# hermanjakobsen/robotic-ultrasound-imaging

Measured on AMD Instinct MI355X. Metric: env-steps/sec (whole node) at 4096 envs/GPU, random-action rollout, higher is better.
Workload: dtype f32

## Files before the change

robotic-ultrasound-imaging_amd/csrc/usim_step16.h:

```cpp
#pragma once
#include <type_traits>

namespace usim {

template <int N, class F>
DI void static_for(F&& f) {
    if constexpr (N > 0) { static_for<N - 1>(f); f(std::integral_constant<int, N - 1>{}); }
}

template <int CTRL>
DI float dpp0(float v) { return __int_as_float(__builtin_amdgcn_update_dpp(0, __float_as_int(v), CTRL, 0xf, 0xf, true)); }
template <int G> DI int glane() { return (int)(threadIdx.x & (G - 1)); }
template <int G, int K> DI float rbc(float v) {
    if constexpr (G == 16) return dpp0<0x150 + K>(v);
    else {
        const int iv = __float_as_int(v);
        const int t = __builtin_amdgcn_update_dpp(iv, iv, 0x150 + K, 0xf, 0x3, false);
        return __int_as_float(__builtin_amdgcn_update_dpp(t, iv, 0x150 + 8 + K, 0xf, 0xc, false));
    }
}
template <int G, int D> DI float rshr0(float v) {
    const float t = dpp0<0x110 + D>(v);
    if constexpr (G == 16) return t; else return (glane<G>() < D) ? 0.f : t;
}
// ... 93 lines not shown
            "v_fmac_f32_dpp %0, %3, %9 row_newbcast:%13 row_mask:0xf bank_mask:0xf\n\t" "v_fmac_f32_dpp %0, %4, %10 row_newbcast:%13 row_mask:0xf bank_mask:0xf\n\t"
            "v_fmac_f32_dpp %0, %5, %11 row_newbcast:%13 row_mask:0xf bank_mask:0xf\n\t" "v_fmac_f32_dpp %0, %6, %12 row_newbcast:%13 row_mask:0xf bank_mask:0xf"
            : "=&v"(s) : "v"(z.x), "v"(z.y), "v"(z.z), "v"(vo.x), "v"(vo.y), "v"(vo.z), "v"(n.x), "v"(n.y), "v"(n.z), "v"(f.x), "v"(f.y), "v"(f.z), "n"(K));
    } else {
        asm("s_nop 1\n\t"
            "v_mul_f32_dpp %0, %1, %7 row_newbcast:%13 row_mask:0xf bank_mask:0x3\n\t"   "v_mul_f32_dpp %0, %1, %7 row_newbcast:%14 row_mask:0xf bank_mask:0xc\n\t"
            "v_fmac_f32_dpp %0, %2, %8 row_newbcast:%13 row_mask:0xf bank_mask:0x3\n\t"  "v_fmac_f32_dpp %0, %2, %8 row_newbcast:%14 row_mask:0xf bank_mask:0xc\n\t"
            "v_fmac_f32_dpp %0, %3, %9 row_newbcast:%13 row_mask:0xf bank_mask:0x3\n\t"  "v_fmac_f32_dpp %0, %3, %9 row_newbcast:%14 row_mask:0xf bank_mask:0xc\n\t"
            "v_fmac_f32_dpp %0, %4, %10 row_newbcast:%13 row_mask:0xf bank_mask:0x3\n\t" "v_fmac_f32_dpp %0, %4, %10 row_newbcast:%14 row_mask:0xf bank_mask:0xc\n\t"
            "v_fmac_f32_dpp %0, %5, %11 row_newbcast:%13 row_mask:0xf bank_mask:0x3\n\t" "v_fmac_f32_dpp %0, %5, %11 row_newbcast:%14 row_mask:0xf bank_mask:0xc\n\t"
            "v_fmac_f32_dpp %0, %6, %12 row_newbcast:%13 row_mask:0xf bank_mask:0x3\n\t" "v_fmac_f32_dpp %0, %6, %12 row_newbcast:%14 row_mask:0xf bank_mask:0xc"
            : "=&v"(s) : "v"(z.x), "v"(z.y), "v"(z.z), "v"(vo.x), "v"(vo.y), "v"(vo.z), "v"(n.x), "v"(n.y), "v"(n.z), "v"(f.x), "v"(f.y), "v"(f.z), "n"(K), "n"(K + 8));
    }
    return s;
}

template <int G>
DI void fk16(const float* at, const float q, f3& X, f3& Y, f3& Z, f3& P) {
    float s, c;
    sincos_(q, s, c);
    const f3 f0 = mk(at[AT_RFIX], at[AT_RFIX + 1], at[AT_RFIX + 2]), f1 = mk(at[AT_RFIX + 3], at[AT_RFIX + 4], at[AT_RFIX + 5]);
    X = f0 * c + f1 * s; Y = f1 * c - f0 * s; Z = mk(at[AT_RFIX + 6], at[AT_RFIX + 7], at[AT_RFIX + 8]);
    P = mk(at[AT_LPOS], at[AT_LPOS + 1], at[AT_LPOS + 2]);
    static_for<3>([&](auto Dc) {
        constexpr int D = 1 << decltype(Dc)::value;
        const f3 LX = mk(rshr<G, D>(X.x, 1.f), rshr<G, D>(X.y, 0.f), rshr<G, D>(X.z, 0.f));
        const f3 LY = mk(rshr<G, D>(Y.x, 0.f), rshr<G, D>(Y.y, 1.f), rshr<G, D>(Y.z, 0.f));
        const f3 LZ = mk(rshr<G, D>(Z.x, 0.f), rshr<G, D>(Z.y, 0.f), rshr<G, D>(Z.z, 1.f));
        const f3 LP = mk(rshr0<G, D>(P.x), rshr0<G, D>(P.y), rshr0<G, D>(P.z));
        const f3 nX = LX * X.x + LY * X.y + LZ * X.z, nY = LX * Y.x + LY * Y.y + LZ * Y.z, nZ = LX * Z.x + LY * Z.y + LZ * Z.z;
        P = LP + LX * P.x + LY * P.y + LZ * P.z;
        X = nX; Y = nY; Z = nZ;
    });
}

DI void jacobian_rows(float* xl, const int gl, const float* Jc, float* Jr) {
    if (gl < 8) {
#pragma unroll
        for (int a = 0; a < 6; ++a) xl[a * 8 + gl] = Jc[a];
    }
    group_sync();
    int arow = (gl & 7) - ((gl & 4) ? 1 : 0);
    arow = arow > 5 ? 5 : arow;
    const float4 j0 = *reinterpret_cast<const float4*>(&xl[arow * 8]), j1 = *reinterpret_cast<const float4*>(&xl[arow * 8 + 4]);
    Jr[0] = j0.x; Jr[1] = j0.y; Jr[2] = j0.z; Jr[3] = j0.w; Jr[4] = j1.x; Jr[5] = j1.y; Jr[6] = j1.z; Jr[7] = j1.w;
}

template <int G>
DI float solve6_task(float* A, float b, const int gl) {
    static_for<6>([&](auto Kc) {
        constexpr int k = decltype(Kc)::value;
        constexpr int lk = TASK_LANE[k];
        const float g = (A[k] - (gl == lk ? 1.f : 0.f)) * rcp_(rbc<G, lk>(A[k]));
#pragma unroll
        for (int c = k + 1; c < 6; ++c) A[c] = fmaf(-g, rbc<G, lk>(A[c]), A[c]);
        b = fmaf(-g, rbc<G, lk>(b), b);
    });
    return b;
}

constexpr int X16_WORDS = 64;
constexpr int X16_RIGID_STRIDE = 84;

#ifndef USIM_WPR16
#define USIM_WPR16 4
#endif
#ifndef USIM_WPR8
#define USIM_WPR8 4
#endif
template <int G> constexpr int wpr() { return G == 16 ? USIM_WPR16 : USIM_WPR8; }
constexpr int MB_POSE = X16_WORDS;
constexpr int MB_OP = MB_POSE + 12;
constexpr int MB_W = MB_OP + 64;
constexpr int MB_Q = MB_W + 16;
constexpr int MB_GOAL = MB_Q + 100;
#ifndef USIM_DRAW_AHEAD
#define USIM_DRAW_AHEAD 1
#endif
constexpr bool DRAW_AHEAD = USIM_DRAW_AHEAD != 0;
#ifndef USIM_LIST_AHEAD
#define USIM_LIST_AHEAD 0
#endif
constexpr bool LIST_AHEAD = USIM_LIST_AHEAD != 0;
constexpr int MB_ACT = MB_GOAL + 12;
constexpr int X2_STRIDE = MB_ACT + (DRAW_AHEAD ? 8 : 0);
template <int G> constexpr int x2_base() { return TB_WORDS + (64 * wpr<G>() / G) * GE_STRIDE; }
static_assert(x2_base<16>() % 4 == 0 && x2_base<8>() % 4 == 0 && X2_STRIDE % 4 == 0 && MB_OP % 4 == 0 && MB_W % 4 == 0 && MB_ACT % 4 == 0, "mailbox block: 16-byte accesses");
static_assert((x2_base<8>() + 32 * X2_STRIDE) * 4 <= 160 * 1024, "split kernel with 8-lane groups: LDS of a CU");
#ifndef USIM_ARM_CULL16
#define USIM_ARM_CULL16 0
#endif
template <int G> constexpr int arm_cull_rounds() { return G == 16 ? USIM_ARM_CULL16 : 7; }

#if defined(USIM_TSTAMP) || defined(USIM_TSTAMP_NOWAIT)
#define USIM_BAR() do { __syncthreads(); ++nbar; } while (0)
#else
#define USIM_BAR() __syncthreads()
#endif


constexpr int ARM_LDS_WORDS = A16_LANES * AT_STRIDE;
template <int TORSO, int ROLE, int G> constexpr int arm_lds_base();
template <int NE, class WR = NoWarm>
struct Carry {
    float dqj, qdj, q0j;
    Episode ep;
    float s[NE], sd[NE];
    WR wr;
};

template <int TORSO, int ROLE, int G> constexpr int arm_lds_base() {
    return ROLE != 0 ? x2_base<G>() + (64 * wpr<G>() / G) * X2_STRIDE : (TORSO ? SOFT16_LDS_WORDS : 16 * X16_RIGID_STRIDE);
}
static_assert((arm_lds_base<1, 1, 8>() + ARM_LDS_WORDS) * 4 <= 160 * 1024 && arm_lds_base<1, 1, 8>() % 4 == 0 && arm_lds_base<1, 1, 16>() % 4 == 0 && arm_lds_base<1, 0, 16>() % 4 == 0
              && arm_lds_base<0, 0, 16>() % 4 == 0, "arm table behind the LDS blocks of every 16-lane kernel");

template <int TORSO, int MODE, int ROLE, int NT, int G = 16, bool RES = false, class WR = NoWarm, bool AHEAD = false>
DI void step16_one(float* lds, const DevModel& M, const DevCfg& C, float* __restrict__ st, const int n, const int npad, const DevIO& io, const int flags, const long long rstep,
                   const bool first_pass, const int sub, const bool more, int& nbar, Carry<TORSO ? (N_TOP + G - 1) / G : 1, WR>& cy) {
    static_assert(!AHEAD || (ROLE == 1 && RES), "action drawn ahead: the arm wave of a resident split launch");
    constexpr bool WARM = !std::is_same<WR, NoWarm>::value;
    static_assert(!WARM || (TORSO == 1 && ROLE == 0) || (TORSO == 1 && MODE == 0), "warm start: the soft-torso kernels");
    constexpr int WPR = (ROLE != 0) ? wpr<G>() : 4;
    constexpr int EPW = 64 / G, EPB = WPR * EPW;
    static_assert(!RES || MODE == 0, "resident state: step launches only");
    constexpr int X2_BASE = x2_base<G>();
    constexpr unsigned GMASK = (G == 16) ? 0xffffu : 0xffu;
    static_assert(G == 16 || (TORSO == 1 && MODE == 0 && ROLE != 0), "8-lane groups: the split soft-torso step only");
    constexpr int NE = TORSO ? (N_TOP + G - 1) / G : 1;
    static_assert(ROLE == 0 || (TORSO == 1 && MODE == 0), "the split kernel is the soft-torso step");
    const int lane = threadIdx.x & 63, wave = (threadIdx.x >> 6) & (WPR - 1);
    constexpr bool RES_HERE = RES && !(ROLE == 2 && G == 16);
    const bool fresh = !RES_HERE || first_pass;
    const int gl = lane & (G - 1), ge = lane / G;
    const int gbase = lane - gl;
    const int eb = wave * EPW + ge;
    const bool auto_reset = (flags & LF_AUTO_RESET) != 0;
    unsigned long long* const dbg = io.dbg;
    const bool refill = (MODE == 1) && io.refill != 0;
    const int item_cnt = refill ? io.count[0] : 1;
    const int item_first = refill ? (int)blockIdx.x * EPB : 0;
    for (int item0 = item_first; item0 < item_cnt; item0 += refill ? (int)gridDim.x * EPB : 1) {
    int env = blockIdx.x * EPB + eb;
    bool valid = env < n;
    int item_ep = 0;
    if (refill) {
        valid = item0 + eb < item_cnt;
        const int2 it = valid ? io.items[item0 + eb] : make_int2(0, 0);
        env = it.x; item_ep = it.y;
    }
    const bool store = valid && gl == 0;
    const int ei = valid ? env : (refill ? 0 : n - 1);
#define LAT(w) st[(size_t)F_LAT * npad + (size_t)ei * LAT_ENV_WORDS + (w)]
#define EB(off) lds[TB_WORDS + eb * GE_STRIDE + (off)]
    float* const warm_rows = st + warm_index(io.bank_row0, npad, (size_t)ei);
    int mbo = X2_BASE + eb * X2_STRIDE;
    if constexpr (ROLE != 0) asm volatile("" : "+v"(mbo));
    float* const xl = (ROLE != 0) ? &lds[mbo]
                                  : (TORSO ? &lds[TB_WORDS + eb * GE_STRIDE + GE_WS] : &lds[eb * X16_RIGID_STRIDE]);
    static_assert(GE_WS + X16_WORDS <= GE_STRIDE, "transpose scratch overlays the wrench records");
    constexpr int GOAL_OFF = (ROLE != 0) ? MB_GOAL : (TORSO ? GE_CG + (MAXCAND + 1) * CG_WORDS - GE_WS : X16_WORDS);
    static_assert(GE_CG + (MAXCAND + 1) * CG_WORDS + 12 <= GE_STRIDE && X16_WORDS + 12 <= X16_RIGID_STRIDE, "room for the goal");
    float* const goal_lds = xl + GOAL_OFF;

    USIM_STAMP(dbg, 0);
    if constexpr (ROLE == 1) { if (dbg && blockIdx.x == 0 && threadIdx.x == 0) dbg[20] = __builtin_readcyclecounter(); }

    float at[AT_STRIDE];
    {
        constexpr int ARM_LDS = arm_lds_base<TORSO, ROLE, G>();
        const float4* ap = fresh ? reinterpret_cast<const float4*>(M.tables + TB_ARM + gl * AT_STRIDE) : reinterpret_cast<const float4*>(lds + ARM_LDS + gl * AT_STRIDE);
        if (fresh) {
#pragma unroll
            for (int v = 0; v < AT_STRIDE / 4; ++v) { const float4 x = ap[v]; at[4 * v] = x.x; at[4 * v + 1] = x.y; at[4 * v + 2] = x.z; at[4 * v + 3] = x.w; }
            if constexpr (RES && ROLE != 2) {
                if (lane < G) {
#pragma unroll
                    for (int v = 0; v < AT_STRIDE / 4; ++v) reinterpret_cast<float4*>(lds + ARM_LDS + gl * AT_STRIDE)[v] = make_float4(at[4 * v], at[4 * v + 1], at[4 * v + 2], at[4 * v + 3]);
                }
            }
        } else {
            const float4* lp = reinterpret_cast<const float4*>(lds + ARM_LDS + gl * AT_STRIDE);
#pragma unroll
            for (int v = 0; v < AT_STRIDE / 4; ++v) { const float4 x = lp[v]; at[4 * v] = x.x; at[4 * v + 1] = x.y; at[4 * v + 2] = x.z; at[4 * v + 3] = x.w; }
        }
    }
    const float* const sp = st + scalar_index(0, (size_t)ei);
    const bool jlane = at[AT_JOINT] != 0.f;
    const int jl = jlane ? gl : NJ - 1;
    float &dqj = cy.dqj, &qdj = cy.qdj, &q0j = cy.q0j;
    Episode& E = cy.ep;
    f3 &ts = E.ts, &te = E.te;
    float &u0 = E.u0, &vbar = E.vbar, &fzbar = E.fzbar, &fzprev = E.fzprev, &dfz = E.dfz, &kst = E.kst, &kdmp = E.kdmp, &mu = E.mu, &epret = E.epret;
    int &t = E.t, &touched = E.touched, &episode = E.episode, &status = E.status;
    float (&s_pre)[NE] = cy.s, (&sd_pre)[NE] = cy.sd;
    if (fresh) {
        dqj = sp[F_Q + jl]; qdj = sp[F_QD + jl]; q0j = sp[F_Q0 + jl];
        float sv[20];
        {
            const float4* s4 = reinterpret_cast<const float4*>(sp + 20);
#pragma unroll
            for (int v = 0; v < 5; ++v) { const float4 x = s4[v]; sv[4 * v] = x.x; sv[4 * v + 1] = x.y; sv[4 * v + 2] = x.z; sv[4 * v + 3] = x.w; }
        }
#define SV(f) sv[(f) - 20]
        ts = mk(SV(F_TS), SV(F_TS + 1), SV(F_TS + 2)); te = mk(SV(F_TE), SV(F_TE + 1), SV(F_TE + 2));
        u0 = SV(F_U0); vbar = SV(F_VBAR); fzbar = SV(F_FZBAR); fzprev = SV(F_FZPREV); dfz = SV(F_DFZ);
        kst = SV(F_KST); kdmp = SV(F_KDMP); mu = SV(F_MU); epret = SV(F_EPRET);
        t = __float_as_int(SV(F_T)); touched = __float_as_int(SV(F_TOUCH)); episode = __float_as_int(SV(F_EPISODE)); status = __float_as_int(SV(F_STATUS));
#undef SV
#pragma unroll
        for (int i = 0; i < NE; ++i) {
            const int e = gl + i * G;
            s_pre[i] = 0.f; sd_pre[i] = 0.f;
            if (TORSO && MODE == 0 && ROLE != 1 && e < N_TOP) { s_pre[i] = LAT(LAT_S + e); sd_pre[i] = LAT(LAT_SD + e); }
            if (TORSO && MODE == 0 && ROLE == 1 && e < N_TOP) s_pre[i] = LAT(LAT_S + e);
        }
        if constexpr (WARM && MODE == 0 && ROLE != 1) warm_load(warm_rows, gl, cy.wr);
    } else if constexpr (RES && ROLE == 1) {
#pragma unroll
        for (int i = 0; i < NE; ++i) { const int e = gl + i * G; s_pre[i] = (e < N_TOP) ? EB(GE_S + e) : 0.f; }
    } else if constexpr (RES && ROLE == 2) {
        const float4 nx = *reinterpret_cast<const float4*>(&lds[mbo + MB_W]);
        if (nx.w != 0.f) {
            kst = nx.x; kdmp = nx.y; mu = nx.z; t = 0;
#pragma unroll
            for (int i = 0; i < NE; ++i) { s_pre[i] = 0.f; sd_pre[i] = 0.f; }
            warm_clear(cy.wr);
        }
    }
    if (!jlane) { dqj = 0.f; qdj = 0.f; q0j = 0.f; }
    float qj = q0j + dqj;
    if (TORSO != 0 && item0 == item_first && first_pass) {
        const float4* src = reinterpret_cast<const float4*>(M.tables);
        float4* dst = reinterpret_cast<float4*>(lds);
        constexpr int NV = TB_WORDS / 4, PER = (NV + NT - 1) / NT;
        float4 tmp[PER];
        int tix = threadIdx.x;
        asm volatile("" : "+v"(tix));
#pragma unroll
        for (int i = 0; i < PER; ++i) { int idx = tix + i * NT; tmp[i] = (idx < NV) ? src[idx] : make_float4(0, 0, 0, 0); }
#pragma unroll
        for (int i = 0; i < PER; ++i) { int idx = tix + i * NT; if (idx < NV) dst[idx] = tmp[i]; }
        USIM_BAR();
    }
    USIM_STAMP(dbg, 1);

    if (MODE == 0 && sub == 0) t += 1;
    const bool last_sub = sub == C.substeps - 1;
    const int tphys = (MODE == 0) ? (t - 1) * C.substeps + sub : 0;
    const float dt = C.dt, inv_h = rcp_((float)C.horizon);
#if defined(USIM_TSTAMP) || defined(USIM_TSTAMP_NOWAIT)
#define RSTAMP(k) do { if (dbg && blockIdx.x == 0 && (threadIdx.x & (64 * WPR - 1)) == 0) dbg[(ROLE == 2 ? 30 : 20) + (k)] = __builtin_readcyclecounter(); } while (0)
#else
#define RSTAMP(k) do { } while (0)
#endif
#define XSTAMP(k) RSTAMP(20 + (k))
    if constexpr (ROLE == 2) {
        RSTAMP(0);
        float* const mb = &lds[mbo];
        const int* tb_shell = reinterpret_cast<const int*>(lds + TB_SHELL);
        float dz, vz, az;
        torso_motion(C, tphys, dz, vz, az);
        lattice_rhs<G, NE>(lds, eb, gl, M, az, kst, kdmp, true, s_pre, sd_pre);
        lattice_solve<G>(lds, eb, gl, gbase);
        RSTAMP(1);
        USIM_BAR();
        RSTAMP(2);
        const f3 xs = mk(mb[MB_POSE], mb[MB_POSE + 1], mb[MB_POSE + 2]), sy = mk(mb[MB_POSE + 3], mb[MB_POSE + 4], mb[MB_POSE + 5]),
                 sz = mk(mb[MB_POSE + 6], mb[MB_POSE + 7], mb[MB_POSE + 8]);
        const f3 sxc = cross(sy, sz);
        int nq = __float_as_int(mb[MB_POSE + 10]);
#pragma unroll
        for (int i = arm_cull_rounds<G>(); i < NE; ++i) {
            const int eraw = i * G + gl, e = eraw < N_TOP ? eraw : N_TOP - 1;
            const bool cand = (eraw < N_TOP) && collide_cull(lds, e, M, C, s_pre[i], dz, xs, sxc, sz);
            const unsigned gm = (unsigned)(__ballot(cand) >> gbase) & GMASK;
            mb[MB_Q + (cand ? nq + __popc(gm & ((1u << gl) - 1u)) : 99)] = __int_as_float(e);
            nq += __popc(gm);
        }
        group_sync();
#if defined(USIM_TSTAMP) || defined(USIM_TSTAMP_NOWAIT)
        if (dbg && blockIdx.x == 0 && wave == 0 && gl == 0) dbg[54 + ge] = 1ull + (unsigned long long)nq;
#endif
        int nc = 0;
        collide_queue<G>(lds, mb + MB_Q, nq, &EB(GE_CG), gl, gbase, M, C, &EB(GE_S), dz, xs, sxc, sy, sz, nc);
        constexpr bool EARLY = G == 8;
        ContactRows P;
        constexpr bool LIST_EARLY = EARLY || (G == 16 && LIST_AHEAD);
        int nc_early = nc, overflow_early = 0, ncmax_early = 0, cel_early[MAXC];
        if constexpr (LIST_EARLY) {
            contact_overflow<G>(lds, eb, gl, gbase, nc_early);
            if (nc_early > MAXC) { overflow_early = 1; nc_early = MAXC; }
            group_sync();
            if constexpr (G == 16) {
                const int m01 = max(__builtin_amdgcn_readlane(nc_early, 0), __builtin_amdgcn_readlane(nc_early, 16));
                const int m23 = max(__builtin_amdgcn_readlane(nc_early, 32), __builtin_amdgcn_readlane(nc_early, 48));
                ncmax_early = max(m01, m23);
            } else {
#pragma unroll
                for (int k = MAXC; k >= 1; --k) if (ncmax_early == 0 && __any(nc_early >= k)) ncmax_early = k;
            }
#pragma unroll
            for (int k = 0; k < MAXC; ++k) cel_early[k] = (k < nc_early) ? __float_as_int(EB(GE_CG + k * CG_WORDS + 6)) : 0;
            if constexpr (EARLY) { if (ncmax_early > 0) contact_rows<G>(lds, eb, gl, M, C, nc_early, cel_early, vz, P); }
        }
        RSTAMP(3);
        USIM_BAR();
        RSTAMP(4);
        if constexpr (!LIST_EARLY) contact_overflow<G>(lds, eb, gl, gbase, nc);
        int overflow = 0;
        if (nc > MAXC) { overflow = 1; nc = MAXC; }
        if constexpr (!LIST_EARLY) group_sync();
        XSTAMP(0);
        int ncmax = 0;
        if constexpr (LIST_EARLY) { nc = nc_early; overflow = overflow_early; ncmax = ncmax_early; }
        else {
#pragma unroll
            for (int k = MAXC; k >= 1; --k) if (ncmax == 0 && __any(nc >= k)) ncmax = k;
        }
        XSTAMP(1);
        float gf[MAXC], W[6] = {0, 0, 0, 0, 0, 0};
        int cel[MAXC];
#pragma unroll
        for (int k = 0; k < MAXC; ++k) { const int ek = __float_as_int(EB(GE_CG + k * CG_WORDS + 6)); gf[k] = 0.f; cel[k] = LIST_EARLY ? cel_early[k] : ((k < nc) ? ek : 0); }
        if (ncmax > 0) {
            float alpha[6], vs[6], Lp[21];
#pragma unroll
            for (int a = 0; a < 6; ++a) {
                alpha[a] = mb[MB_OP + 48 + a]; vs[a] = mb[MB_OP + 54 + a];
#pragma unroll
                for (int b = 0; b <= a; ++b) Lp[PK(a, b)] = mb[MB_OP + a * 8 + b];
            }
            XSTAMP(2);
            contact_solve<G, EARLY, true>(lds, eb, gl, M, C, nc, ncmax, cel, Lp, alpha, vs, mu, vz, P, W, gf, dbg, cy.wr);
            XSTAMP(3);
        } else warm_clear(cy.wr);
        if (gl == 0) {
            *reinterpret_cast<float4*>(&mb[MB_W]) = make_float4(W[0], W[1], W[2], W[3]);
            *reinterpret_cast<float4*>(&mb[MB_W + 4]) = make_float4(W[4], W[5], __int_as_float(nc), __int_as_float(overflow));
#pragma unroll
            for (int k = 0; k < MAXC; ++k) { const int sh = tb_shell[cel[k]]; mb[MB_W + 8 + k] = __int_as_float((k < nc) ? sh : -1); }
        }
        RSTAMP(5);
        USIM_BAR();
        RSTAMP(6);
        {
            float acc_e[NE];
#pragma unroll
            for (int i = 0; i < NE; ++i) { const int e = gl + i * G; acc_e[i] = (e < N_TOP) ? EB(GE_A + e) : 0.f; }
#pragma unroll
            for (int k = 0; k < MAXC; ++k) {
#pragma unroll
                for (int i = 0; i < NE; ++i) {
                    const int e = (gl + i * G < N_TOP) ? gl + i * G : N_TOP - 1;
                    acc_e[i] = fmaf(lds[TB_LINV + e * LROW + cel[k]], gf[k], acc_e[i]);
                }
            }
#pragma unroll
            for (int i = 0; i < NE; ++i) {
                const int e = gl + i * G;
                if (e >= N_TOP) continue;
                const float sdn = sd_pre[i] + dt * acc_e[i];
                const float sn = s_pre[i] + dt * sdn;
                if (valid) { LAT(LAT_SD + e) = sdn; LAT(LAT_S + e) = sn; }
                if constexpr (RES) { sd_pre[i] = sdn; s_pre[i] = sn; EB(GE_S + e) = sn; }
            }
            if constexpr (WARM) { if (valid) warm_store(warm_rows, gl, cy.wr); }
        }
        RSTAMP(7);
        USIM_BAR();
        RSTAMP(8);
        return;
    }
    const int comp = gl & 3;
    const bool blk = (gl & 4) != 0;
    const bool is_task = (gl < 8) && comp != 3;
    auto pick = [&](f3 v) { return comp == 0 ? v.x : (comp == 1 ? v.y : v.z); };

    bool need = false;
    int ep_t = episode;
    if constexpr (MODE == 1) {
        need = refill ? valid : (io.mask ? io.mask[ei] != 0 : true);
        if (!__any(need)) continue;
        ep_t = refill ? item_ep : episode + 1;
        if (!refill) episode = ep_t;
        const uint32_t gid = (uint32_t)(C.env_offset + ei);
        const u4 r = philox(gid, (uint32_t)ep_t, (uint32_t)(gl < 3 ? gl : 2), 0u, C.key0, C.key1);
        const float ra = __uint_as_float(r.a), rb = __uint_as_float(r.b), rc = __uint_as_float(r.c), rd = __uint_as_float(r.d);
        u4 A, B, Cc;
        A.a = __float_as_uint(rbc<G, 0>(ra)); A.b = __float_as_uint(rbc<G, 0>(rb)); A.c = __float_as_uint(rbc<G, 0>(rc)); A.d = __float_as_uint(rbc<G, 0>(rd));
        B.a = __float_as_uint(rbc<G, 1>(ra)); B.b = __float_as_uint(rbc<G, 1>(rb)); B.c = __float_as_uint(rbc<G, 1>(rc)); B.d = __float_as_uint(rbc<G, 1>(rd));
        Cc.a = __float_as_uint(rbc<G, 2>(ra)); Cc.b = __float_as_uint(rbc<G, 2>(rb)); Cc.c = __float_as_uint(rbc<G, 2>(rc)); Cc.d = __float_as_uint(rbc<G, 2>(rd));
        const float tz = M.torso[2] + M.base[2] + C.top_off;
        f3 noise = mk(0, 0, 0);
        kst = C.stiffness; kdmp = C.damping;
        if (io.reset_params) {
            const float* p = io.reset_params + (size_t)ei * 13;
            ts = mk(p[0], p[1], p[2]); te = mk(p[3], p[4], p[5]); u0 = p[6]; noise = mk(p[7], p[8], p[9]);
            kst = p[10]; kdmp = p[11]; mu = p[12];
        } else {
            if (C.det_traj) { ts = mk(0.062f, -0.020f, 0.896f); te = mk(-0.032f, -0.075f, 0.896f); }
            else {
                const float tx = M.torso[0] + M.base[0], ty = M.torso[1] + M.base[1];
                const float xs0 = -0.15f + tx + 0.03f, xstep = (0.15f + tx - xs0) / 49.f;
                const float ys0 = -C.y_range + ty, ystep = 2.f * C.y_range / 49.f;
                ts = mk(xs0 + (float)urange(A.a, 50u) * xstep, ys0 + (float)urange(A.b, 50u) * ystep, tz);
                te = mk(xs0 + (float)urange(A.c, 50u) * xstep, ys0 + (float)urange(A.d, 50u) * ystep, tz);
            }
            u0 = u01(B.a);
            if (C.rand_pos) {
                const float r1 = sqrtf(-2.f * logf(u01_open(B.b))), th1 = 2.f * PI_F * u01(B.c);
                const float r2 = sqrtf(-2.f * logf(u01_open(B.d))), th2 = 2.f * PI_F * u01(Cc.a);
                noise = mk(r1 * cosf(th1) * 0.0025f, r1 * sinf(th1) * 0.0025f, r2 * cosf(th2) * 0.010f);
            }
            if (C.rand_solref) { kst = 1300.f + (float)urange(Cc.b, 300u); kdmp = 17.f + (float)urange(Cc.c, 24u); }
            float pf = C.probe_fric;
            if (C.rand_fric) pf *= 0.5f + 1.5f * u01(Cc.d);
            mu = fmaxf(pf, C.elem_fric);
            if (C.probe_geoms == 2 && !C.pair) mu = 0.5f * (mu + fmaxf(C.probe_fric2, C.elem_fric));
        }
        const float uu = clampf(u0, 0.f, 1.f);
        const f3 tp0 = ts + (te - ts) * uu;
        const f3 target = mk(tp0.x + noise.x + M.ikb[0] - M.base[0], tp0.y + noise.y + M.ikb[1] - M.base[1], tp0.z + noise.z + M.ikb[2] - M.base[2]);
        const f3 gx = mk(M.grot[0], M.grot[3], M.grot[6]), gy = mk(M.grot[1], M.grot[4], M.grot[7]), gz = mk(M.grot[2], M.grot[5], M.grot[8]);
// ... 335 lines not shown
                draw_action(rstep + 1, nxt);
                keep_action(nxt);
            }
        }
        RSTAMP(5);
        USIM_BAR();
        RSTAMP(6);
        const float4 w0 = *reinterpret_cast<const float4*>(&xl[MB_W]), w1 = *reinterpret_cast<const float4*>(&xl[MB_W + 4]);
        W[0] = w0.x; W[1] = w0.y; W[2] = w0.z; W[3] = w0.w; W[4] = w1.x; W[5] = w1.y;
        ncon = __float_as_int(w1.z); overflow = __float_as_int(w1.w);
#pragma unroll
        for (int k = 0; k < MAXC; ++k) con_shell[k] = __float_as_int(xl[MB_W + 8 + k]);
    } else if constexpr (TORSO != 0) {
        const int* tb_shell = reinterpret_cast<const int*>(lds + TB_SHELL);
        float dz, vz, az;
        torso_motion(C, tphys, dz, vz, az);
        lattice_rhs<G, NE>(lds, eb, gl, M, az, kst, kdmp, MODE == 0, s_pre, sd_pre);
        USIM_STAMP(dbg, 5);
        int nc = collide_all<G, NE>(lds, eb, gl, gbase, M, C, MODE == 0, s_pre, dz, xs, sy, sz);
        lattice_solve<G>(lds, eb, gl, gbase);
        contact_overflow<G>(lds, eb, gl, gbase, nc);
        USIM_STAMP(dbg, 7);
        if (nc > MAXC) { overflow = 1; nc = MAXC; }
        ncon = nc;
        group_sync();
        int ncmax = 0;
#pragma unroll
        for (int k = MAXC; k >= 1; --k) if (ncmax == 0 && __any(nc >= k)) ncmax = k;
        float gf[MAXC];
        int cel[MAXC];
#pragma unroll
        for (int k = 0; k < MAXC; ++k) { gf[k] = 0.f; cel[k] = (k < nc) ? __float_as_int(EB(GE_CG + k * CG_WORDS + 6)) : 0; }
        if (ncmax > 0) {
            float alpha[6], vs[6], Lp[21];
            static_for<6>([&](auto Ac) {
                constexpr int a = decltype(Ac)::value;
                alpha[a] = rbc<G, TASK_LANE[a]>(alpha_t); vs[a] = rbc<G, TASK_LANE[a]>(v6);
#pragma unroll
                for (int b = 0; b <= a; ++b) Lp[PK(a, b)] = rbc<G, TASK_LANE[a]>(Li[b]);
            });
            USIM_STAMP(dbg, 8);
            if constexpr (MODE == 0) contact_solve<G, false, false>(lds, eb, gl, M, C, nc, ncmax, cel, Lp, alpha, vs, mu, vz, ContactRows{}, W, gf, dbg, cy.wr);
            else { NoWarm cold; contact_solve<G, false, false>(lds, eb, gl, M, C, nc, ncmax, cel, Lp, alpha, vs, mu, vz, ContactRows{}, W, gf, dbg, cold); }
        } else warm_clear(cy.wr);
        USIM_STAMP(dbg, 11);
        if constexpr (MODE == 1) {
            if (valid && need && !refill) {
                for (int e = gl; e < N_TOP; e += G) { LAT(LAT_S + e) = 0.f; LAT(LAT_SD + e) = 0.f; }
                if constexpr (WARM) warm_rows_clear<G>(warm_rows, gl);
            }
        } else {
            float acc_e[NE];
#pragma unroll
            for (int i = 0; i < NE; ++i) { const int e = gl + i * G; acc_e[i] = (e < N_TOP) ? EB(GE_A + e) : 0.f; }
#pragma unroll
            for (int k = 0; k < MAXC; ++k) {
                if (k < ncmax) {
#pragma unroll
                    for (int i = 0; i < NE; ++i) {
                        const int e = (gl + i * G < N_TOP) ? gl + i * G : N_TOP - 1;
                        acc_e[i] = fmaf(lds[TB_LINV + e * LROW + cel[k]], gf[k], acc_e[i]);
                    }
                }
            }
#pragma unroll
            for (int i = 0; i < NE; ++i) {
                const int e = gl + i * G;
                if (e >= N_TOP) continue;
                const float sdn = sd_pre[i] + dt * acc_e[i];
                const float sn = s_pre[i] + dt * sdn;
                if (valid) { LAT(LAT_SD + e) = sdn; LAT(LAT_S + e) = sn; }
                if constexpr (RES) { sd_pre[i] = sdn; s_pre[i] = sn; }
            }
            if constexpr (WARM) { if (valid) warm_store(warm_rows, gl, cy.wr); }
        }
#pragma unroll
        for (int k = 0; k < MAXC; ++k) con_shell[k] = (k < nc) ? tb_shell[cel[k]] : -1;
    }
    USIM_STAMP(dbg, 12);

    if constexpr (ROLE != 1) precompute();
    float tq[3];
    f3 hv;
    {
        float qacc = qs, aq_t = alpha_t;
        if (TORSO) {
#pragma unroll
            for (int a = 0; a < 6; ++a) { qacc = fmaf(Xm[a], W[a], qacc); aq_t = fmaf(Li[a], W[a], aq_t); }
        }
        float aq[6];
        static_for<6>([&](auto Ac) { constexpr int a = decltype(Ac)::value; aq[a] = rbc<G, TASK_LANE[a]>(aq_t); });
        const f3 alq = mk(aq[3], aq[4], aq[5]);
        const f3 alt = al + alq;
        const f3 a7 = ao + mk(aq[0], aq[1], aq[2]) - cross(alq, s_xso);
        const f3 ac = a7 + cross(alt, s_rc) + s_wwrc;
        const f3 N = rot_inertia(alt) + s_nw;
        const f3 Fp = ac * PROBE_MASS;
        const f3 tw = N + cross(s_arm, Fp) - mk(W[3], W[4], W[5]);
        tq[0] = rbc<G, NJ - 1>(dot(sx, tw)); tq[1] = rbc<G, NJ - 1>(dot(sy, tw)); tq[2] = rbc<G, NJ - 1>(dot(sz, tw));
        USIM_STAMP(dbg, 13);
        hv = mk(0, 0, 0);
        if constexpr (MODE == 0) {
            const float xk = row_times_joint<G, NJ>(Mi, qacc);
            const float rhs = fmaf(-dt * JOINT_DAMP, xk, qacc);
            qdj = fmaf(dt, rhs, qdj); dqj = fmaf(dt, qdj, dqj);
            if (!jlane) { qdj = 0.f; dqj = 0.f; }
            qj = q0j + dqj;
            const float v2_t = row_times_joint<G, NJ>(Jr, qdj);
            float v2[6];
            static_for<6>([&](auto Ac) { constexpr int a = decltype(Ac)::value; v2[a] = rbc<G, TASK_LANE[a]>(v2_t); });
            hv = mk(v2[0], v2[1], v2[2]) + cross(mk(v2[3], v2[4], v2[5]), hand - xs);
        }
    }
    USIM_STAMP(dbg, 14);

    bool done = false;
    {
        if (MODE == 1) fzbar = W[2];
        obs[0] = W[0]; obs[1] = W[1]; obs[2] = W[2];
        obs[3] = tq[0]; obs[4] = tq[1]; obs[5] = tq[2];
        obs[6] = hv.x; obs[7] = hv.y; obs[8] = hv.z;
        obs[9] = fzbar - 5.0f; obs[10] = dfz - 0.0f; obs[11] = vbar - 0.04f;
        if constexpr (MODE == 1) {
            if (overflow) status |= 1;
            if (refill) {
                if (valid && need) {
                    const int sl = ep_t & (BANK_DEPTH - 1);
                    if (jlane) BK(sl, BQ0 + gl) = qj;
                    if (gl == 0) {
                        BK(sl, BTS) = ts.x; BK(sl, BTS + 1) = ts.y; BK(sl, BTS + 2) = ts.z; BK(sl, BTE) = te.x; BK(sl, BTE + 1) = te.y; BK(sl, BTE + 2) = te.z;
                        BK(sl, BU0) = u0; BK(sl, BKST) = kst; BK(sl, BKDMP) = kdmp; BK(sl, BMU) = mu; BK(sl, BFZ) = fzbar;
#pragma unroll
                        for (int a = 0; a < OBS_DIM; ++a) BK(sl, BOBS + a) = obs[a];
                        BKI(sl, BSTATUS) = overflow ? 1 : 0;
                    }
                }
            } else if (store && io.obs && need) {
#pragma unroll
                for (int a = 0; a < OBS_DIM; ++a) io.obs[(size_t)ei * OBS_DIM + a] = obs[a];
            }
        } else if (last_sub) {
        const bool contact = ncon > 0;
        if (contact) touched = 1;
        const float force_rew = contact ? force_e : 0.f, dforce_rew = contact ? dforce_e : 0.f;
        float reward = pos_rew + ori_rew + vel_rew + force_rew + dforce_rew;
        done = t >= C.horizon;
        const float hvn = sqrt_(dot(hv, hv));
        vbar += (hvn - vbar) * rcp_((float)t);
        const float fz = W[2];
        dfz = (fz - fzprev) * rcp_(C.dt_ctrl);
        fzprev = fz;
        fzbar = 0.1f * fz + 0.9f * fzbar;
        const bool jviol = (qj < at[AT_QMIN] + 0.1f) || (qj > at[AT_QMAX] - 0.1f);
        const unsigned jany = (unsigned)(__ballot(jviol) >> gbase) & GMASK;
        if (C.early_term) {
            const bool term = (jany != 0u) || (pos_err_norm > 1.0f) || (contact && ori_err > 0.10f) || (touched && !contact);
            done = done || term;
        }
        epret += reward;
        if (io.log && valid) {
            float* L = io.log + (size_t)ei * LOG_WIDTH;
            if (jlane) L[26 + gl] = qj;
            if (gl == 0) {
                const float upn = clampf((float)t * inv_h + u0, 0.f, 1.f);
                const f3 tpn = ts + (te - ts) * upn;
                L[0] = xw.x; L[1] = xw.y; L[2] = xw.z; L[3] = tpn.x; L[4] = tpn.y; L[5] = tpn.z;
                L[6] = hv.x; L[7] = hv.y; L[8] = hv.z; L[9] = 0.04f; L[10] = vbar;
                L[11] = qe[0]; L[12] = qe[1]; L[13] = qe[2]; L[14] = qe[3];
                L[15] = M.gquat[0]; L[16] = M.gquat[1]; L[17] = M.gquat[2]; L[18] = M.gquat[3];
                L[19] = ori_err * 5.0f;
                L[20] = fz; L[21] = 5.0f; L[22] = fzbar; L[23] = dfz; L[24] = 0.f; L[25] = contact ? 1.f : 0.f;
                L[40] = (float)(t - 1) * inv_h * 100.f;
                L[41] = pos_rew; L[42] = ori_rew; L[43] = vel_rew; L[44] = force_rew; L[45] = dforce_rew;
            }
        }
        if (overflow) status |= 1;
        {
            const float chk = rbc<G, 7>(prefix_sum<G>(fabsf(qj) + 1e-3f * fabsf(qdj)));
            if (!(chk < 1.0e3f)) { status |= 4; done = true; epret -= reward; reward = 0.f; if (!(epret == epret)) epret = 0.f; }
        }
        if (store) {
            io.rew[ei] = reward;
            if (io.status_out) io.status_out[ei] = status;
            io.done[ei] = done ? 1 : 0;
            if (io.contacts) {
                io.contacts[(size_t)ei * (1 + MAXC)] = ncon;
#pragma unroll
                for (int k = 0; k < MAXC; ++k) io.contacts[(size_t)ei * (1 + MAXC) + 1 + k] = con_shell[k];
            }
            if (done) {
                if (io.term_obs) {
#pragma unroll
                    for (int a = 0; a < OBS_DIM; ++a) io.term_obs[(size_t)ei * OBS_DIM + a] = obs[a];
                }
                if (io.ep_ret) io.ep_ret[ei] = epret;
                if (io.ep_len) io.ep_len[ei] = t;
            }
        }
        need = done && auto_reset;
        if (store && io.obs && !need) {
#pragma unroll
            for (int a = 0; a < OBS_DIM; ++a) io.obs[(size_t)ei * OBS_DIM + a] = obs[a];
        }
        }
    }

    if constexpr (ROLE == 1) { RSTAMP(7); USIM_BAR(); RSTAMP(8); }
    if (MODE == 0 && need) {
        episode += 1;
        const int sl = episode & (BANK_DEPTH - 1);
        qj = jlane ? BK(sl, BQ0 + jl) : 0.f; q0j = qj; qdj = 0.f; dqj = 0.f;
        ts = mk(BK(sl, BTS), BK(sl, BTS + 1), BK(sl, BTS + 2)); te = mk(BK(sl, BTE), BK(sl, BTE + 1), BK(sl, BTE + 2));
        u0 = BK(sl, BU0); kst = BK(sl, BKST); kdmp = BK(sl, BKDMP); mu = BK(sl, BMU); fzbar = BK(sl, BFZ);
        episode_begin(E, BKI(sl, BSTATUS));
        if (store && io.obs) {
#pragma unroll
            for (int a = 0; a < OBS_DIM; ++a) io.obs[(size_t)ei * OBS_DIM + a] = BK(sl, BOBS + a);
        }
        if (TORSO && valid) for (int e = gl; e < N_TOP; e += G) { LAT(LAT_S + e) = 0.f; LAT(LAT_SD + e) = 0.f; }
        if constexpr (WARM) {
            if (valid) warm_rows_clear<G>(warm_rows, gl);
            warm_clear(cy.wr);
        }
        if constexpr (RES && TORSO != 0) {
#pragma unroll
            for (int i = 0; i < NE; ++i) {
                s_pre[i] = 0.f; sd_pre[i] = 0.f;
                if (ROLE == 1 && gl + i * G < N_TOP) EB(GE_S + gl + i * G) = 0.f;
            }
        }
        if (store) order_refill(io, env, episode);
    }
    if constexpr (RES && ROLE == 1) {
        if (gl == 0) *reinterpret_cast<float4*>(&xl[MB_W]) = make_float4(kst, kdmp, mu, (MODE == 0 && need) ? 1.f : 0.f);
    }
    USIM_STAMP(dbg, 15);

    if (valid && (MODE == 0 || (need && !refill))) {
        float* const so = st + scalar_index(0, (size_t)ei);
        if (jlane) {
            so[F_Q + gl] = dqj; so[F_QD + gl] = qdj;
            if (need) so[F_Q0 + gl] = q0j;
        }
        if (gl == 0) {
            float4* s4 = reinterpret_cast<float4*>(so);
            if (need) {
                so[F_TS] = ts.x; so[F_TS + 1] = ts.y; so[F_TS + 2] = ts.z;
                s4[6] = make_float4(te.x, te.y, te.z, u0);
            }
            s4[7] = make_float4(vbar, fzbar, fzprev, dfz);
            s4[8] = make_float4(kst, kdmp, mu, __int_as_float(t));
            s4[9] = make_float4(__int_as_float(touched), __int_as_float(episode), epret, __int_as_float(status));
        }
    }
    if (refill) group_sync();
    }
    if (MODE == 1 && refill) work_list_close(io);
    USIM_STAMP(dbg, 16);
    if constexpr (ROLE == 1) RSTAMP(9);
#undef RSTAMP
#undef XSTAMP
#undef LAT
#undef EB
}

template <int TORSO, int MODE, int ROLE, int NT, bool MULTI = false, int G = 16, class WR = NoWarm, bool ACTS = false>
DI void step16_body(float* lds, const DevModel& M, const DevCfg& C, float* __restrict__ st, const int n, const int npad, const DevIO& io0, const int flags, const long long rstep) {
    const int S = (MULTI && MODE == 0 && C.substeps > 1) ? C.substeps : 1;
    const int nsub = (MULTI && MODE == 0) ? (io0.nsub > 1 ? io0.nsub : 1) * S : 1;
    DevIO io = io0;
    int nbar = 0;
    Carry<TORSO ? (N_TOP + G - 1) / G : 1, WR> cy;
    int sub = 0;
    long long cstep = rstep;
    for (int ks = 0; ks < nsub; ++ks) {
        constexpr bool AHEAD = DRAW_AHEAD && ROLE == 1 && MULTI && MODE == 0 && !ACTS;
        step16_one<TORSO, MODE, ROLE, NT, G, MULTI && MODE == 0, WR, AHEAD>(lds, M, C, st, n, npad, io, flags, cstep, ks == 0, sub, ks + 1 < nsub, nbar, cy);
        const bool ctrl_done = sub == S - 1;
        if (ctrl_done) { sub = 0; ++cstep; } else ++sub;
        if (ks + 1 < nsub) {
            __threadfence_block();
            if constexpr (ROLE != 0) USIM_BAR();
            if (io0.block && ctrl_done) advance_rollout_block(io, (size_t)n, C.adim);
            if constexpr (ACTS) { if (ctrl_done) io.act += (size_t)n * C.adim; }
        }
    }
#if defined(USIM_TSTAMP) || defined(USIM_TSTAMP_NOWAIT)
    if (ROLE != 0 && io0.dbg && blockIdx.x == 0 && (threadIdx.x & (64 * wpr<G>() - 1)) == 0) io0.dbg[ROLE == 1 ? 46 : 47] = (unsigned long long)nbar;
#endif
}

template <int TORSO, int OCC, int MODE, bool MULTI = false, bool WARM = false>
__global__ __launch_bounds__(256) __attribute__((amdgpu_waves_per_eu(OCC, OCC))) void usim_step16_kernel(const DevModel M, const DevCfg C, float* __restrict__ st, int n, int npad,
                                                                                                          const DevIO io, int flags, long long rstep) {
    extern __shared__ __attribute__((aligned(16))) float lds[];
    step16_body<TORSO, MODE, 0, 256, MULTI, 16, typename std::conditional<WARM, WarmOf<16>::type, NoWarm>::type>(lds, M, C, st, n, npad, io, flags, rstep);
}

template <int TORSO, int OCC, bool WARM = false>
__global__ __launch_bounds__(256) __attribute__((amdgpu_waves_per_eu(OCC, OCC))) void usim_step16_acts_kernel(const DevModel M, const DevCfg C, float* __restrict__ st, int n, int npad,
                                                                                                               const DevIO io, int flags, long long rstep) {
    extern __shared__ __attribute__((aligned(16))) float lds[];
    step16_body<TORSO, 0, 0, 256, true, 16, typename std::conditional<WARM, WarmOf<16>::type, NoWarm>::type, true>(lds, M, C, st, n, npad, io, flags, rstep);
}

template <bool MULTI, int G = 16, bool WARM = false>
__global__ __launch_bounds__(128 * wpr<G>()) __attribute__((amdgpu_waves_per_eu(2, 2))) void usim_step32_kernel(const DevModel* __restrict__ Mp, const DevCfg* __restrict__ Cp, float* __restrict__ st, int n, int npad,
                                                                                                                  const DevIO io, int flags, long long rstep) {
    extern __shared__ __attribute__((aligned(16))) float lds[];
    const DevModel& M = *Mp; const DevCfg& C = *Cp;
    constexpr int NT = 128 * wpr<G>();
    typedef typename std::conditional<WARM, typename WarmOf<G>::type, NoWarm>::type WR;
    if (threadIdx.x < NT / 2) step16_body<1, 0, 1, NT, MULTI, G, WR>(lds, M, C, st, n, npad, io, flags, rstep);
    else step16_body<1, 0, 2, NT, MULTI, G, WR>(lds, M, C, st, n, npad, io, flags, rstep);
}

template <int G = 16, bool WARM = false>
__global__ __launch_bounds__(128 * wpr<G>()) __attribute__((amdgpu_waves_per_eu(2, 2))) void usim_step32_acts_kernel(const DevModel* __restrict__ Mp, const DevCfg* __restrict__ Cp, float* __restrict__ st, int n, int npad,
                                                                                                                       const DevIO io, int flags, long long rstep) {
    extern __shared__ __attribute__((aligned(16))) float lds[];
    const DevModel& M = *Mp; const DevCfg& C = *Cp;
    constexpr int NT = 128 * wpr<G>();
    typedef typename std::conditional<WARM, typename WarmOf<G>::type, NoWarm>::type WR;
    if (threadIdx.x < NT / 2) step16_body<1, 0, 1, NT, true, G, WR, true>(lds, M, C, st, n, npad, io, flags, rstep);
    else step16_body<1, 0, 2, NT, true, G, WR, true>(lds, M, C, st, n, npad, io, flags, rstep);
}

}
```

Measured before the change: 237.0 million.

## Decide episode reset early in arm wave to drop inter-substep barrier

For the split kernel with 8-lane groups, the arm role now runs the Euler joint update first and computes the termination checks (limit ballot, runaway sum, early-term conditions) right away. It then publishes the next episode's stiffness, damping and friction plus the reset flag to the mailbox before the kinematics. This lets the barrier between substeps in the body loop be removed and moves the mid-step barrier to a configurable point; the contact wave also publishes shell ids earlier. The goal is fewer block-wide barriers per step and more overlap between roles, at the cost of more complex barrier placement and the risk of LDS mailbox ordering races.

```diff
diff --git a/robotic-ultrasound-imaging_amd/csrc/usim_step16.h b/robotic-ultrasound-imaging_amd/csrc/usim_step16.h
--- a/robotic-ultrasound-imaging_amd/csrc/usim_step16.h
+++ b/robotic-ultrasound-imaging_amd/csrc/usim_step16.h
@@ -199,6 +199,30 @@
 #define USIM_LIST_AHEAD 0
 #endif
 constexpr bool LIST_AHEAD = USIM_LIST_AHEAD != 0;
+#ifndef USIM_EARLY_EPISODE16
+#define USIM_EARLY_EPISODE16 0
+#endif
+#ifndef USIM_EARLY_EPISODE8
+#define USIM_EARLY_EPISODE8 1
+#endif
+template <int G> constexpr bool early_episode() { return (G == 16 ? USIM_EARLY_EPISODE16 : USIM_EARLY_EPISODE8) != 0; }
+#ifndef USIM_BAR4_16
+#define USIM_BAR4_16 0
+#endif
+#ifndef USIM_BAR4_8
+#define USIM_BAR4_8 2
+#endif
+#ifndef USIM_LAT_CARRY16
+#define USIM_LAT_CARRY16 1
+#endif
+template <int G> constexpr int bar4_at() { return G == 16 ? USIM_BAR4_16 : USIM_BAR4_8; }
+#ifndef USIM_SHELL_EARLY16
+#define USIM_SHELL_EARLY16 0
+#endif
+#ifndef USIM_SHELL_EARLY8
+#define USIM_SHELL_EARLY8 1
+#endif
+template <int G> constexpr bool shell_early() { return (G == 16 ? USIM_SHELL_EARLY16 : USIM_SHELL_EARLY8) != 0; }
 constexpr int MB_ACT = MB_GOAL + 12;
 constexpr int X2_STRIDE = MB_ACT + (DRAW_AHEAD ? 8 : 0);
 template <int G> constexpr int x2_base() { return TB_WORDS + (64 * wpr<G>() / G) * GE_STRIDE; }
@@ -247,7 +271,11 @@
     constexpr int NE = TORSO ? (N_TOP + G - 1) / G : 1;
     static_assert(ROLE == 0 || (TORSO == 1 && MODE == 0), "the split kernel is the soft-torso step");
     const int lane = threadIdx.x & 63, wave = (threadIdx.x >> 6) & (WPR - 1);
-    constexpr bool RES_HERE = RES && !(ROLE == 2 && G == 16);
+    constexpr bool EARLY_EP = early_episode<G>() && RES && ROLE != 0;
+    constexpr bool SHELL_EARLY = shell_early<G>();
+    constexpr bool RES_HERE = RES && (EARLY_EP || !(ROLE == 2 && G == 16));
+    constexpr bool LAT_REREAD = EARLY_EP && ROLE == 2 && G == 16 && USIM_LAT_CARRY16 == 0;
+    constexpr int BAR4_AT = EARLY_EP ? bar4_at<G>() : 2;
     const bool fresh = !RES_HERE || first_pass;
     const int gl = lane & (G - 1), ge = lane / G;
     const int gbase = lane - gl;
@@ -343,6 +371,12 @@
 #pragma unroll
             for (int i = 0; i < NE; ++i) { s_pre[i] = 0.f; sd_pre[i] = 0.f; }
             warm_clear(cy.wr);
+        } else if constexpr (LAT_REREAD) {
+#pragma unroll
+            for (int i = 0; i < NE; ++i) {
+                const int e = gl + i * G;
+                if (e < N_TOP) { s_pre[i] = LAT(LAT_S + e); sd_pre[i] = LAT(LAT_SD + e); }
+            }
         }
     }
     if (!jlane) { dqj = 0.f; qdj = 0.f; q0j = 0.f; }
@@ -374,6 +408,9 @@
 #define XSTAMP(k) RSTAMP(20 + (k))
     if constexpr (ROLE == 2) {
         RSTAMP(0);
+#if defined(USIM_TSTAMP) || defined(USIM_TSTAMP_NOWAIT)
+        if (dbg && blockIdx.x == 0 && (threadIdx.x & (64 * WPR - 1)) == 0 && !first_pass) dbg[39] = dbg[36];
+#endif
         float* const mb = &lds[mbo];
         const int* tb_shell = reinterpret_cast<const int*>(lds + TB_SHELL);
         float dz, vz, az;
@@ -440,6 +477,11 @@
         int cel[MAXC];
 #pragma unroll
         for (int k = 0; k < MAXC; ++k) { const int ek = __float_as_int(EB(GE_CG + k * CG_WORDS + 6)); gf[k] = 0.f; cel[k] = LIST_EARLY ? cel_early[k] : ((k < nc) ? ek : 0); }
+        auto publish_shells = [&]() {
+#pragma unroll
+            for (int k = 0; k < MAXC; ++k) { const int sh = tb_shell[cel[k]]; mb[MB_W + 8 + k] = __int_as_float((k < nc) ? sh : -1); }
+        };
+        if constexpr (SHELL_EARLY) { if (gl == 0) publish_shells(); }
         if (ncmax > 0) {
             float alpha[6], vs[6], Lp[21];
 #pragma unroll
@@ -455,8 +497,7 @@
         if (gl == 0) {
             *reinterpret_cast<float4*>(&mb[MB_W]) = make_float4(W[0], W[1], W[2], W[3]);
             *reinterpret_cast<float4*>(&mb[MB_W + 4]) = make_float4(W[4], W[5], __int_as_float(nc), __int_as_float(overflow));
-#pragma unroll
-            for (int k = 0; k < MAXC; ++k) { const int sh = tb_shell[cel[k]]; mb[MB_W + 8 + k] = __int_as_float((k < nc) ? sh : -1); }
+            if constexpr (!SHELL_EARLY) publish_shells();
         }
         RSTAMP(5);
         USIM_BAR();
@@ -958,11 +999,42 @@
     if constexpr (ROLE != 1) precompute();
     float tq[3];
     f3 hv;
+#define LIMIT_BALLOT(jany) const bool jviol = (qj < at[AT_QMIN] + 0.1f) || (qj > at[AT_QMAX] - 0.1f); jany = (unsigned)(__ballot(jviol) >> gbase) & GMASK
+#define RUNAWAY_SUM() rbc<G, 7>(prefix_sum<G>(fabsf(qj) + 1e-3f * fabsf(qdj)))
+    unsigned jany_early = 0u;
+    float chk_early = 0.f;
     {
         float qacc = qs, aq_t = alpha_t;
         if (TORSO) {
 #pragma unroll
             for (int a = 0; a < 6; ++a) { qacc = fmaf(Xm[a], W[a], qacc); aq_t = fmaf(Li[a], W[a], aq_t); }
+        }
+#define EULER_STEP() do { \
+            const float xk = row_times_joint<G, NJ>(Mi, qacc); \
+            const float rhs = fmaf(-dt * JOINT_DAMP, xk, qacc); \
+            qdj = fmaf(dt, rhs, qdj); dqj = fmaf(dt, qdj, dqj); \
+            if (!jlane) { qdj = 0.f; dqj = 0.f; } \
+            qj = q0j + dqj; } while (0)
+        if constexpr (EARLY_EP) {
+            EULER_STEP();
+            bool need_early = false;
+            float kst_n = kst, kdmp_n = kdmp, mu_n = mu;
+            if (last_sub) {
+                { LIMIT_BALLOT(jany_early); }
+                chk_early = RUNAWAY_SUM();
+                const bool contact = ncon > 0;
+                bool over = t >= C.horizon;
+                if (C.early_term) over = over || (jany_early != 0u) || (pos_err_norm > 1.0f) || (contact && ori_err > 0.10f) || (touched && !contact);
+                over = over || !(chk_early < 1.0e3f);
+                need_early = over && auto_reset;
+                if (need_early) {
+                    const int sl = (episode + 1) & (BANK_DEPTH - 1);
+                    kst_n = BK(sl, BKST); kdmp_n = BK(sl, BKDMP); mu_n = BK(sl, BMU);
+                }
+            }
+            if (gl == 0) *reinterpret_cast<float4*>(&xl[MB_W]) = make_float4(kst_n, kdmp_n, mu_n, need_early ? 1.f : 0.f);
+            RSTAMP(7);
+            if constexpr (BAR4_AT == 0) { USIM_BAR(); RSTAMP(8); }
         }
         float aq[6];
         static_for<6>([&](auto Ac) { constexpr int a = decltype(Ac)::value; aq[a] = rbc<G, TASK_LANE[a]>(aq_t); });
@@ -977,17 +1049,14 @@
         USIM_STAMP(dbg, 13);
         hv = mk(0, 0, 0);
         if constexpr (MODE == 0) {
-            const float xk = row_times_joint<G, NJ>(Mi, qacc);
-            const float rhs = fmaf(-dt * JOINT_DAMP, xk, qacc);
-            qdj = fmaf(dt, rhs, qdj); dqj = fmaf(dt, qdj, dqj);
-            if (!jlane) { qdj = 0.f; dqj = 0.f; }
-            qj = q0j + dqj;
+            if constexpr (!EARLY_EP) EULER_STEP();
             const float v2_t = row_times_joint<G, NJ>(Jr, qdj);
             float v2[6];
             static_for<6>([&](auto Ac) { constexpr int a = decltype(Ac)::value; v2[a] = rbc<G, TASK_LANE[a]>(v2_t); });
             hv = mk(v2[0], v2[1], v2[2]) + cross(mk(v2[3], v2[4], v2[5]), hand - xs);
         }
     }
+    if constexpr (ROLE == 1 && BAR4_AT == 1) { USIM_BAR(); RSTAMP(8); }
     USIM_STAMP(dbg, 14);
 
     bool done = false;
@@ -1027,8 +1096,8 @@
         dfz = (fz - fzprev) * rcp_(C.dt_ctrl);
         fzprev = fz;
         fzbar = 0.1f * fz + 0.9f * fzbar;
-        const bool jviol = (qj < at[AT_QMIN] + 0.1f) || (qj > at[AT_QMAX] - 0.1f);
-        const unsigned jany = (unsigned)(__ballot(jviol) >> gbase) & GMASK;
+        unsigned jany = jany_early;
+        if constexpr (!EARLY_EP) { LIMIT_BALLOT(jany); }
         if (C.early_term) {
             const bool term = (jany != 0u) || (pos_err_norm > 1.0f) || (contact && ori_err > 0.10f) || (touched && !contact);
             done = done || term;
@@ -1052,7 +1121,7 @@
         }
         if (overflow) status |= 1;
         {
-            const float chk = rbc<G, 7>(prefix_sum<G>(fabsf(qj) + 1e-3f * fabsf(qdj)));
+            const float chk = EARLY_EP ? chk_early : RUNAWAY_SUM();
             if (!(chk < 1.0e3f)) { status |= 4; done = true; epret -= reward; reward = 0.f; if (!(epret == epret)) epret = 0.f; }
         }
         if (store) {
@@ -1081,7 +1150,9 @@
         }
     }
 
-    if constexpr (ROLE == 1) { RSTAMP(7); USIM_BAR(); RSTAMP(8); }
+    if constexpr (ROLE == 1 && EARLY_EP && BAR4_AT == 2) { RSTAMP(28); USIM_BAR(); RSTAMP(8); }
+    if constexpr (ROLE == 1 && !EARLY_EP) { RSTAMP(7); USIM_BAR(); RSTAMP(8); }
+    if constexpr (ROLE == 1 && EARLY_EP && BAR4_AT != 2) RSTAMP(28);
     if (MODE == 0 && need) {
         episode += 1;
         const int sl = episode & (BANK_DEPTH - 1);
@@ -1107,7 +1178,7 @@
         }
         if (store) order_refill(io, env, episode);
     }
-    if constexpr (RES && ROLE == 1) {
+    if constexpr (RES && ROLE == 1 && !EARLY_EP) {
         if (gl == 0) *reinterpret_cast<float4*>(&xl[MB_W]) = make_float4(kst, kdmp, mu, (MODE == 0 && need) ? 1.f : 0.f);
     }
     USIM_STAMP(dbg, 15);
@@ -1136,6 +1207,9 @@
     if constexpr (ROLE == 1) RSTAMP(9);
 #undef RSTAMP
 #undef XSTAMP
+#undef LIMIT_BALLOT
+#undef RUNAWAY_SUM
+#undef EULER_STEP
 #undef LAT
 #undef EB
 }
@@ -1155,8 +1229,9 @@
         const bool ctrl_done = sub == S - 1;
         if (ctrl_done) { sub = 0; ++cstep; } else ++sub;
         if (ks + 1 < nsub) {
-            __threadfence_block();
-            if constexpr (ROLE != 0) USIM_BAR();
+            constexpr bool MEET = ROLE != 0 && !early_episode<G>();
+            if constexpr (ROLE == 0 || MEET) __threadfence_block();
+            if constexpr (MEET) USIM_BAR();
             if (io0.block && ctrl_done) advance_rollout_block(io, (size_t)n, C.adim);
             if constexpr (ACTS) { if (ctrl_done) io.act += (size_t)n * C.adim; }
         }
```

Result: no change. 237.0 million (median of 2 runs) (+0.0%).
